# ben-hayes/neural-waveshaping-synthesis

Measured on AMD Instinct MI355X. Metric: audio_samples_per_sec, higher is better.
Workload: dtype f32 (fp16x2-split MFMA contractions = 22-bit products, fp32 accumulate; FiLM interpolation bf16x3-split MFMA = exact fp32 operands); 1 GPU; NEWT forward, vn checkpoint, FastNEWT LUT, batch 64/GPU x 500 frames (4 s @ 16 kHz), torch.rand F0/control, RNG draws on device; batch_per_gpu=64, frames=500, samples_per_utterance=64000, parallelism=batch-shard x1, exciter_opts=0, streams=2

## Files before the change

include/nws_hip.h:

```cpp
#ifndef NWS_HIP_H
#define NWS_HIP_H

#include <stddef.h>
#include <stdint.h>

#ifdef __cplusplus
extern "C" {
#endif

#define NWS_ABI_VERSION 6

#define NWS_N_HARMONICS 101
#define NWS_N_SHAPERS 64
#define NWS_HIDDEN 128
#define NWS_HOP 128
#define NWS_FIR_LEN 256
#define NWS_N_BANDS 129
#define NWS_FIR_HALF 128
#define NWS_SHAPER_WIDTH 8
#define NWS_FILM_CH 256

enum {
  NWS_OK = 0,
  NWS_ERR_UNSUPPORTED = -1,
// ... 85 lines not shown
#define NWS_MLP_FRAGS_BYTES 1474560
int nws_mlp_frags(const NwsWeights* w, const float* fir_design , void* frags_out, void* stream);

int nws_fir_design_matrix(const float* window , float* D_out, void* stream);

#define NWS_SPEC_ROW 132
#define NWS_MLP_SPEC_BYTES 200704
#define NWS_MLP_SPEC_FOLD_FLOATS 49668
int nws_fir_spectrum_map(const float* fir_design , double* S_out );
int nws_mlp_spec_fold(const float* proj_w, const float* proj_b, const float* newt_w0, const float* newt_b0, const float* hgen_w0,
                      const float* hgen_b0, const float* hgen_w3 , const float* hgen_b3 ,
                      const double* S , float* folded_out );
int nws_mlp_spec_frags(const float* folded , void* frags , void* stream);
int nws_frame_mlps_spec_serves(const NwsWeights* w, int B, int T);
int nws_frame_mlps_spec(const NwsWeights* w, const float* gru_out, int B, int T, float* film_out, float* spec_out, void* stream);

int nws_fir_noise(const float* fir , const float* noise , const float* add_in ,
                  int B, int T, float* out , void* stream);
int nws_fir_noise_window(const float* fir, const float* noise, int noise_len, int origin, const float* add_in, int B, int T,
                         float* out, void* stream);
int nws_fir_noise_spec(const float* spec , const float* noise , const float* add_in ,
                       int B, int T, float* out , void* stream);

int nws_fir_noise_grad(const float* noise , const float* grad_out , int B, int T,
                       float* grad_fir , void* stream);
int nws_fir_from_h_grad(const float* grad_fir , const float* fir_design , int B, int T,
                        float* grad_H , void* stream);
int nws_sum_batch_time(const float* x , int B, int C, int T, float* out , void* stream);

typedef struct NwsReverbPlan {
// ... 369 lines not shown
```

include/nws_hip_debug.h:

```cpp
#ifndef NWS_HIP_DEBUG_H
#define NWS_HIP_DEBUG_H
#include "nws_hip.h"
#ifdef __cplusplus
extern "C" {
#endif

int nws_debug_frame_mlps_kernel(int mode);

int nws_debug_forward_spec(int on);

int nws_debug_queue_busy(int groups, int spin_us, float* sink , void* stream);

int nws_debug_generic_exciter_plan(const NwsGenericModel* model, int B, int T, int out[8]);

int nws_debug_generic_gru_plan(int hidden, int C_in, int out[4]);

#ifdef __cplusplus
}
#endif
#endif
```

neural-waveshaping-synthesis_amd/_lib.py:

```python
from __future__ import annotations

import ctypes as C
import os

_HERE = os.path.dirname(os.path.abspath(__file__))
LIB_PATH = os.path.join(_HERE, "libnws_hip.so")

PROBE_LIB_PATH = os.path.join(_HERE, "libnws_probe.so")

ABI_VERSION = 6
EXCITER_VALU_FILM = 1
EXCITER_ONE_TERM = 2
EXCITER_HYBRID = 4
EXCITER_HYBRID_W = 8
EXCITER_BANK_NOFRACT = 16
N_HARMONICS = 101
N_SHAPERS = 64
HIDDEN = 128
HOP = 128
FIR_LEN = 256
FIR_HALF = 128
MLP_FRAGS_BYTES = 1474560
MLP_SPEC_BYTES = 200704
MLP_SPEC_FOLD_FLOATS = 49668
# ... 117 lines not shown
    "nws_control_gru_state": (C.c_int, [C.POINTER(NwsWeights), _fp, C.c_int, C.c_int, C.c_int, _fp, _fp, _fp, _fp]),
    "nws_control_gru_carry": (C.c_int, [C.POINTER(NwsWeights), _fp, _fp, C.c_int, C.c_int, C.c_int, _fp, _fp, _fp]),
    "nws_control_gru_batched": (C.c_int, [C.POINTER(NwsWeights), _fp, C.c_int, C.c_int, C.c_int, _fp, _fp, _fp, _fp]),
    "nws_control_gru_grad_workspace_bytes": (C.c_size_t, [C.c_int, C.c_int, C.c_int]),
    "nws_control_gru_grad": (C.c_int, [C.POINTER(NwsWeights), _fp, C.c_int, C.c_int, C.c_int, _fp, _fp, _fp, _fp, _fp, _fp, _fp, _fp,
                                       _fp, _fp, _fp, C.c_size_t, _fp]),
    "nws_frame_mlps": (C.c_int, [C.POINTER(NwsWeights), _fp, _fp, C.c_int, C.c_int, _fp, _fp, _fp, _fp, _fp]),
    "nws_mlp_frags": (C.c_int, [C.POINTER(NwsWeights), _fp, _fp, _fp]),
    "nws_debug_frame_mlps_kernel": (C.c_int, [C.c_int]),
    "nws_debug_forward_spec": (C.c_int, [C.c_int]),
    "nws_fir_spectrum_map": (C.c_int, [_fp, _fp]),
    "nws_mlp_spec_fold": (C.c_int, [_fp, _fp, _fp, _fp, _fp, _fp, _fp, _fp, _fp, _fp]),
    "nws_mlp_spec_frags": (C.c_int, [_fp, _fp, _fp]),
    "nws_frame_mlps_spec_serves": (C.c_int, [C.POINTER(NwsWeights), C.c_int, C.c_int]),
    "nws_frame_mlps_spec": (C.c_int, [C.POINTER(NwsWeights), _fp, C.c_int, C.c_int, _fp, _fp, _fp]),
    "nws_fir_noise_spec": (C.c_int, [_fp, _fp, _fp, C.c_int, C.c_int, _fp, _fp]),
    "nws_fir_design_matrix": (C.c_int, [_fp, _fp, _fp]),
    "nws_fir_noise": (C.c_int, [_fp, _fp, _fp, C.c_int, C.c_int, _fp, _fp]),
    "nws_fir_noise_window": (C.c_int, [_fp, _fp, C.c_int, C.c_int, _fp, C.c_int, C.c_int, _fp, _fp]),
    "nws_fir_noise_grad": (C.c_int, [_fp, _fp, C.c_int, C.c_int, _fp, _fp]),
    "nws_fir_from_h_grad": (C.c_int, [_fp, _fp, C.c_int, C.c_int, _fp, _fp]),
    "nws_sum_batch_time": (C.c_int, [_fp, C.c_int, C.c_int, C.c_int, _fp, _fp]),
    "nws_reverb_linear_chunk": (C.c_int, [C.POINTER(NwsReverbPlan), _fp, _fp, _fp, C.c_int, C.c_int, _fp, _fp, C.c_int, _fp, _fp,
                                          C.c_size_t, _fp]),
    "nws_reverb_plan": (C.c_int, [C.c_int, C.c_int, C.POINTER(NwsReverbPlan)]),
    "nws_reverb_plan_serves": (C.c_int, [C.POINTER(NwsReverbPlan), C.c_int, C.c_int]),
    "nws_reverb_table_bytes": (C.c_size_t, [C.POINTER(NwsReverbPlan)]),
    "nws_reverb_spectrum_bytes": (C.c_size_t, [C.POINTER(NwsReverbPlan)]),
    "nws_reverb_workspace_bytes": (C.c_size_t, [C.POINTER(NwsReverbPlan), C.c_int]),
    "nws_reverb_build_tables": (C.c_int, [C.POINTER(NwsReverbPlan), _fp, _fp]),
# ... 242 lines not shown
```

neural-waveshaping-synthesis_amd/build.py:

```python
import concurrent.futures as cf
import hashlib
import os
import subprocess
import sys

HERE = os.path.dirname(os.path.abspath(__file__))
CSRC = os.path.join(HERE, "csrc")
OBJ = os.path.join(HERE, "csrc", "_obj")
LIB = os.path.join(HERE, "libnws_hip.so")
OPS_LIB = os.path.join(HERE, "libnws_torch_ops.so")
PROBE_LIB = os.path.join(HERE, "libnws_probe.so")
SOURCES = ["exciter_newt.hip", "control_gru.hip", "control_gru_grad.hip", "frame_mlps.hip", "fir_noise.hip", "fir_noise_grad.hip", "reverb_fft.hip", "forward.hip",
           "loudness.hip", "loudness_stream.hip", "loudness_causal.hip", "mfcc.hip", "stft_loss.hip", "stft_grad.hip", "pyin.hip", "pyin_stream.hip", "resample.hip", "resample_stream.hip", "stages.hip", "td_mlp_grad.hip", "newt_grad.hip", "g_newt_grad.hip", "adam_step.hip", "generic.hip", "stream.hip", "queue_probe.hip", "exchange.hip", "grad_reduce.hip", "note_control.hip"]
PROBE_SOURCES = ["coexec_probe.hip"]
FLAGS = ["--offload-arch=gfx950", "-O3", "-std=c++17", "-ffp-contract=off", "-fPIC", "-fvisibility=default",
         "-Wall", "-Wno-unused-function", "-Wno-pass-failed", "-Rpass-analysis=kernel-resource-usage"]
KEEP_SLP = ("control_gru.hip",)
EXTRA_FLAGS = {src: ["-fno-slp-vectorize"] for src in SOURCES + PROBE_SOURCES if src not in KEEP_SLP}
FLAGS += [f for f in os.environ.get("NWS_EXTRA_HIPCC_FLAGS", "").split() if f]
LLVM_BIN = "/opt/rocm/lib/llvm/bin"
SWIZZLE_ALLOW = ("pk_probe_kernel", "pk_probe2_kernel", "pk_probe_mixed_kernel")


def _hipcc():
# ... 87 lines not shown
        else:
            window.append((1, set(), text))
        window = window[-8:]
    return found


REGISTER_BUDGETS = (
    ("exciter_newt_kernelILi4ELi2ELi2E", 80, "default oscillator kernel: three 8-wave workgroups per CU"),
    ("exciter_newt_kernelILi4ELi2ELi6E", 80, "one-term variant: three 8-wave workgroups per CU"),
    ("exciter_newt_kernelILi4ELi2ELi10E", 80, "hybrid variant: three 8-wave workgroups per CU"),
    ("exciter_newt_kernelILi4ELi2ELi26E", 80, "hybrid-W variant: three 8-wave workgroups per CU"),
    ("exciter_newt_kernelILi5ELi1ELi0E", 128, "exact-shaper bank kernel: four 4-wave workgroups per CU (38.8 KB of LDS each)"),
    ("exciter_newt_kernelILi6ELi1ELi0E", 128, "exact-shaper bank kernel (no v_fract): four 4-wave workgroups per CU"),
    ("g_exciter_newt_mfma_kernel", 128, "runtime-size oscillator kernel: four 4-wave workgroups per CU"),
)


def kernel_registers(remarks):
    regs, name = {}, None
    for line in remarks.splitlines():
        if "Function Name:" in line:
            name = line.split("Function Name:")[1].split("[-Rpass")[0].strip()
            regs[name] = 0
        elif name is not None and (" VGPRs:" in line or " AGPRs:" in line) and "Spill" not in line:
            regs[name] += int(line.split("GPRs:")[1].split()[0])
    return regs


def check_register_budgets(remarks, budgets=None):
    over = []
    for kernel, n in kernel_registers(remarks).items():
        for key, budget, why in (REGISTER_BUDGETS if budgets is None else budgets):
            if key in kernel and n > budget:
                over.append((kernel, n, budget, why))
    return over


def build_torch_ops(force=False, verbose=True):
    try:
        import torch
        from torch.utils import cpp_extension as ce
    except Exception as e:
        print(f"torch not importable ({e}): skipping libnws_torch_ops.so", file=sys.stderr)
        return None
    src = os.path.join(CSRC, "torch_ops.cpp")
    h = hashlib.sha256(open(src, "rb").read())
    h.update(open(os.path.join(HERE, "..", "include", "nws_hip.h"), "rb").read())
# ... 95 lines not shown
```

neural-waveshaping-synthesis_amd/csrc/forward.hip:

```cpp
#include "nws_common.h"

namespace {

struct Carve {
  char* p;
  size_t left;
  bool ok = true;
  void* take(size_t bytes) {
    bytes = (bytes + 255) & ~size_t(255);
    if (bytes > left) {
      ok = false;
      return nullptr;
    }
    void* r = p;
    p += bytes;
    left -= bytes;
    return r;
  }
};

size_t aligned(size_t b) { return (b + 255) & ~size_t(255); }

constexpr size_t kFirRow = NWS_SPEC_ROW > NWS_FIR_HALF ? NWS_SPEC_ROW : NWS_FIR_HALF;

// ... 71 lines not shown
                 const Arena& a, void* stream) {
  hipStream_t st = (hipStream_t)stream;
  int rc = NWS_OK;
  if (batched_gru) {
    NWS_STAGE(0, nws_phase_carry(f0, nullptr, B, T, a.carry, stream));
    NWS_STAGE(1, nws_control_gru_batched(w, control, B, C, T, nullptr, a.gru_out, nullptr, stream));
  } else {
    NWS_STAGE(0, NWS_OK);
    NWS_STAGE(1, nws_control_gru_carry(w, control, f0, B, C, T, a.gru_out, a.carry, stream));
  }
  return NWS_OK;
}

int audio_half(const NwsWeights* w, const NwsForwardAux* aux, const float* f0, int B, int T, float sample_rate,
               const float* phase_u, const float* rand_phase, const float* noise, float* out, const Arena& a, void* stream,
               void* wait_before_exciter = nullptr, void* record_after_exciter = nullptr, bool with_reverb = true) {
  hipStream_t st = (hipStream_t)stream;
  int rc = NWS_OK;
  const size_t N = (size_t)T * NWS_HOP;
  const bool spec = nws_frame_mlps_spec_serves(w, B, T) != 0;
  if (spec)
    NWS_STAGE(2, nws_frame_mlps_spec(w, a.gru_out, B, T, a.film, a.fir, stream));
  else
    NWS_STAGE(2, nws_frame_mlps(w, a.gru_out, aux->fir_design, B, T, nullptr, a.film, nullptr, a.fir, stream));
  if (spec)
    NWS_STAGE(4, nws_fir_noise_spec(a.fir, noise, nullptr, B, T, a.noise_out, stream));
  else
    NWS_STAGE(4, nws_fir_noise(a.fir, noise, nullptr, B, T, a.noise_out, stream));
  if (wait_before_exciter != nullptr) {
    const hipError_t e = hipStreamWaitEvent(st, (hipEvent_t)wait_before_exciter, 0);
    if (e != hipSuccess) return (int)e;
  }
  NWS_STAGE(3, nws_exciter_newt_add(w, f0, nullptr, a.carry, phase_u, rand_phase, a.film, a.noise_out, B, T, sample_rate, nullptr, a.pre, stream));
  if (record_after_exciter != nullptr) {
    const hipError_t e = hipEventRecord((hipEvent_t)record_after_exciter, st);
    if (e != hipSuccess) return (int)e;
  }
// ... 28 lines not shown
  const size_t N = (size_t)T * NWS_HOP;
  return aligned((size_t)B * (N / 32) * sizeof(double)) + aligned((size_t)B * T * NWS_HIDDEN * sizeof(float));
}

int nws_forward(const NwsWeights* w, const NwsForwardAux* aux, const float* f0, const float* control, int B, int C,
                int T, float sample_rate, const float* phase_u, const float* rand_phase, const float* noise, float* out,
                void* workspace, size_t workspace_bytes, void* stream) {
  if (!w || !aux_ok(aux)) return NWS_ERR_BAD_ARG;
  if (!f0 || !control || !phase_u || !rand_phase || !noise || !out || !workspace) return NWS_ERR_BAD_ARG;
  if (B <= 0 || T < 2 || C < 2) return NWS_ERR_BAD_ARG;
  if (T > (1 << 23) || !nws_reverb_plan_serves(aux->plan, T * NWS_HOP, 0)) return NWS_ERR_BAD_ARG;
  const Arena a = carve_arena(aux->plan, workspace, workspace_bytes, B, T, false);
  if (!a.ok) return NWS_ERR_WORKSPACE;
  const int rc = control_half(w, f0, control, B, C, T, 0, a, stream);
  if (rc != NWS_OK) return rc;
  return audio_half(w, aux, f0, B, T, sample_rate, phase_u, rand_phase, noise, out, a, stream);
}

int nws_forward_control(const NwsWeights* w, const float* f0, const float* control, int B, int C, int T, int batched_gru,
                        void* workspace, size_t workspace_bytes, void* stream) {
  if (!w || !f0 || !control || !workspace) return NWS_ERR_BAD_ARG;
  if (B <= 0 || T < 2 || C < 2) return NWS_ERR_BAD_ARG;
  const Arena a = carve_arena(nullptr, workspace, workspace_bytes, B, T, true);
  if (!a.ok) return NWS_ERR_WORKSPACE;
  return control_half(w, f0, control, B, C, T, batched_gru, a, stream);
}

int nws_forward_audio(const NwsWeights* w, const NwsForwardAux* aux, const float* f0, int B, int T, float sample_rate,
                      const float* phase_u, const float* rand_phase, const float* noise, float* out, void* workspace,
                      size_t workspace_bytes, void* stream) {
  if (!w || !aux_ok(aux)) return NWS_ERR_BAD_ARG;
// ... 116 lines not shown
```

neural-waveshaping-synthesis_amd/csrc/frame_mlps.hip:

```cpp
#include <cstdlib>

#include "nws_common.h"
#include "mlp_few.h"

namespace {

constexpr int kFT = 32;
constexpr int kXS = 33;
constexpr int kPS = 36;
constexpr int kRows = 132;
constexpr int kDK = 132;
constexpr float kLnEps = 1e-5f;

struct MlpLds {
  float emb[kRows * kXS];
  float p0[kRows * kXS];
  float p1[kRows * kXS];
  float stage[4][kFT * kPS];
  float red[2][4][kFT];
};

template <int KH>
__device__ __forceinline__ void gemm_tile(const float* __restrict__ W, int ldw, int row0, int n_rows,
                                          const float* __restrict__ X, int lane, f32x16& acc) {
// ... 691 lines not shown
  wr_split2(y[2], y[3], h1, l1);
  wr_split2(y[4], y[5], h2, l2);
  wr_split2(y[6], y[7], h3, l3);
  hi = f16x8{h0.x, h0.y, h1.x, h1.y, h2.x, h2.y, h3.x, h3.y};
  lo = f16x8{l0.x, l0.y, l1.x, l1.y, l2.x, l2.y, l3.x, l3.y};
}

__device__ __forceinline__ const char* wr_spec_chunk(const char* frags, int path, int k) {
  if (k == 0) return frags + kT3Base + (size_t)path * 65536;
  if (k == 1) return frags + kT2Base + (size_t)(path ? kT2Kb[1][2] : kT2Kb[0][2]) * 1024;
  if (k == 2) return frags + kT2Base + (size_t)(path ? kT2Kb[1][3] : kT2Kb[0][3]) * 1024;
  if (k == 3) return path ? frags + kT3Base + 131072 : frags + kT2Base + (size_t)kT2Kb[0][4] * 1024;
  return frags + kT2Base + (size_t)kT2Kb[0][5] * 1024;
}

__device__ __forceinline__ void wr_dma(const char* __restrict__ src, char* dst, int kb, int wave, int lane) {
  typedef __attribute__((address_space(1))) const void* gptr_t;
  typedef __attribute__((address_space(3))) void* lptr_t;
  const int per = kb * 128;
  const char* s = src + wave * per + lane * 16;
  char* d = dst + wave * per;
#pragma unroll
  for (int j = 0; j < 8; ++j) __builtin_amdgcn_global_load_lds((gptr_t)(s + j * 1024), (lptr_t)(d + j * 1024), 16, 0, 0);
  if (kb == 72) __builtin_amdgcn_global_load_lds((gptr_t)(s + 8192), (lptr_t)(d + 8192), 16, 0, 0);
}

template <int KS, int NMT, bool TRANSPOSED, bool ZERO = false>
__device__ __forceinline__ void wr_layer_mma(const char* slot, int mt0, const WrAct& x, f32x16* acc, int lane) {
  const char* a = slot + (size_t)mt0 * KS * 2048 + lane * 16;
  constexpr int S = KS * NMT;
  f16x8 wh[3], wl[3];
  auto ld = [&](int s2, int b) {
    const int mt = s2 % NMT, ks = s2 / NMT;
    wh[b] = *reinterpret_cast<const f16x8*>(a + (mt * KS + ks) * 2048);
    wl[b] = *reinterpret_cast<const f16x8*>(a + (mt * KS + ks) * 2048 + 1024);
  };
  ld(0, 0);
  if (S > 1) ld(1, 1);
  __builtin_amdgcn_sched_barrier(0x6);
  __builtin_amdgcn_s_setprio(2);
#pragma unroll
  for (int s2 = 0; s2 < S; ++s2) {
    const int mt = s2 % NMT, ks = s2 / NMT, b = s2 % 3;
    if (s2 + 2 < S) ld(s2 + 2, (s2 + 2) % 3);
    __builtin_amdgcn_sched_barrier(0x6);
    if (!TRANSPOSED) {
      acc[mt] = __builtin_amdgcn_mfma_f32_32x32x16_f16(wh[b], x.lo[ks], (ZERO && ks == 0) ? f32x16{} : acc[mt], 0, 0, 0);
      acc[mt] = __builtin_amdgcn_mfma_f32_32x32x16_f16(wl[b], x.hi[ks], acc[mt], 0, 0, 0);
      acc[mt] = __builtin_amdgcn_mfma_f32_32x32x16_f16(wh[b], x.hi[ks], acc[mt], 0, 0, 0);
    } else {
      acc[mt] = __builtin_amdgcn_mfma_f32_32x32x16_f16(x.lo[ks], wh[b], (ZERO && ks == 0) ? f32x16{} : acc[mt], 0, 0, 0);
      acc[mt] = __builtin_amdgcn_mfma_f32_32x32x16_f16(x.hi[ks], wl[b], acc[mt], 0, 0, 0);
      acc[mt] = __builtin_amdgcn_mfma_f32_32x32x16_f16(x.hi[ks], wh[b], acc[mt], 0, 0, 0);
    }
    __builtin_amdgcn_sched_barrier(0x6);
  }
  __builtin_amdgcn_s_setprio(0);
}

// ... 10 lines not shown
    }
}

__device__ __forceinline__ void wr_pack(const f32x16 (&v)[4], WrAct& out) {
#pragma unroll
  for (int mt = 0; mt < 4; ++mt)
#pragma unroll
    for (int g = 0; g < 2; ++g) {
      float y[8];
#pragma unroll
      for (int i = 0; i < 8; ++i) y[i] = v[mt][8 * g + i];
      wr_pack8(y, out.hi[2 * mt + g], out.lo[2 * mt + g]);
    }
}

__device__ __forceinline__ void wr_layer_norm(f32x16 (&v)[4], const float* g, const float* bt, int half) {
  float s0 = 0.0f, s1 = 0.0f, s2 = 0.0f, s3 = 0.0f;
#pragma unroll
  for (int r = 0; r < 16; ++r) {
    s0 += v[0][r];
    s1 += v[1][r];
    s2 += v[2][r];
    s3 += v[3][r];
  }
  float s = (s0 + s1) + (s2 + s3);
  s += nws_swap_halves(s);
  const float mean = s * (1.0f / NWS_HIDDEN);
  float q0 = 0.0f, q1 = 0.0f, q2 = 0.0f, q3 = 0.0f;
#pragma unroll
  for (int r = 0; r < 16; ++r) {
    v[0][r] -= mean;
    v[1][r] -= mean;
    v[2][r] -= mean;
    v[3][r] -= mean;
    q0 = fmaf(v[0][r], v[0][r], q0);
    q1 = fmaf(v[1][r], v[1][r], q1);
    q2 = fmaf(v[2][r], v[2][r], q2);
    q3 = fmaf(v[3][r], v[3][r], q3);
  }
  float q = (q0 + q1) + (q2 + q3);
  q += nws_swap_halves(q);
  const float rstd = 1.0f / sqrtf(q * (1.0f / NWS_HIDDEN) + kLnEps);
#pragma unroll
  for (int mt = 0; mt < 4; ++mt)
#pragma unroll
    for (int qd = 0; qd < 4; ++qd) {
      const int c = 32 * mt + 8 * qd + 4 * half;
      const float4 g4 = *reinterpret_cast<const float4*>(g + c), b4 = *reinterpret_cast<const float4*>(bt + c);
      const float gg[4] = {g4.x, g4.y, g4.z, g4.w}, bb[4] = {b4.x, b4.y, b4.z, b4.w};
#pragma unroll
      for (int i = 0; i < 4; ++i) {
        const float y = fmaf(v[mt][4 * qd + i] * rstd, gg[i], bb[i]);
        v[mt][4 * qd + i] = fmaxf(y, 0.01f * y);
      }
    }
}

template <int LD, bool BIAS>
__device__ __forceinline__ void wr_store_rows(__amdgpu_buffer_rsrc_t out, const f32x16& acc, int lane_off, int tile, float bias) {
#pragma unroll
  for (int r = 0; r < 16; ++r)
    __builtin_amdgcn_raw_buffer_store_b32(__builtin_bit_cast(unsigned, BIAS ? acc[r] + bias : acc[r]), out,
                                          lane_off + ((r & 3) * LD + 32 * tile) * 4, 8 * (r >> 2) * LD * 4, 0);
}

template <bool TAPS, bool SPEC = false>
__global__ __launch_bounds__(512, 2) void frame_mlps_wr_kernel(NwsWeights w, const float* __restrict__ gru_out, int F, int T,
                                                                 float* __restrict__ emb_out, float* __restrict__ film_out,
                                                                 float* __restrict__ H_out, float* __restrict__ fir_out,
                                                                 const int xcd_blocks = 0) {
  static_assert(!(TAPS && SPEC), "the folded form has neither an embedding nor H to store");
  extern __shared__ __attribute__((aligned(16))) char smem_raw[];
  WrLds& L = *reinterpret_cast<WrLds*>(smem_raw);
  const int tid = threadIdx.x, lane = tid & 63;
  const int wave = __builtin_amdgcn_readfirstlane(tid >> 6);
  const int fb = xcd_blocks > 0 ? (int)(blockIdx.x >> 4) * 8 + (int)(blockIdx.x & 7) : (int)blockIdx.x;
  const int path = xcd_blocks > 0 ? (int)((blockIdx.x >> 3) & 1) : (int)blockIdx.y;
  if (xcd_blocks > 0 && fb >= xcd_blocks) return;
  const int half = lane >> 5, col = lane & 31;
  const int f0 = fb * kWrFrames + 32 * wave;
  const int frame = f0 + col;
  const char* const frags = static_cast<const char*>(w.mlp_frags);
  const char* T2 = frags + kT2Base;
  const float* const spar = reinterpret_cast<const float*>(frags + kT3Base + kT3ParKb * 1024);
  char* const S0 = L.slot[0];
  char* const S1 = L.slot[1];

  wr_dma(SPEC ? wr_spec_chunk(frags, path, 0) : T2 + (size_t)kT2Kb[0][0] * 1024, S0, 64, wave, lane);
  const int grp = wave >> 1, pc = tid & 127;
  float pv[4];
  {
    auto sel4 = [&](const float* a, const float* b, const float* c, const float* d) { return grp == 0 ? a : grp == 1 ? b : grp == 2 ? c : d; };
    const float* const hb0 = SPEC ? spar + 128 * path : path ? w.hgen_b[0] : w.newt_mlp_b[0];
    const float* const hg0 = path ? w.hgen_ln_g[0] : w.newt_ln_g[0];
    const float* const ht0 = path ? w.hgen_ln_b[0] : w.newt_ln_b[0];
    const float* const hb1 = path ? w.hgen_b[1] : w.newt_mlp_b[1];
    const float* const hg1 = path ? w.hgen_ln_g[1] : w.newt_ln_g[1];
    const float* const ht1 = path ? w.hgen_ln_b[1] : w.newt_ln_b[1];
    const float* const hb2 = path ? w.hgen_b[2] : w.newt_mlp_b[2];
    const float* const hg2 = path ? w.hgen_ln_g[2] : w.newt_ln_g[2];
    const float* const ht2 = path ? w.hgen_ln_b[2] : w.newt_ln_b[2];
    const float* const ob = path ? (SPEC ? spar + 256 : w.hgen_b[3]) : w.newt_mlp_b[3];
    const float* const ox = path ? (SPEC ? spar + 384 : w.hgen_w[3] + (size_t)128 * NWS_HIDDEN) : w.newt_mlp_b[3] + 128;
    pv[0] = sel4(w.proj_b, hb0, hg0, ht0)[pc];
    pv[1] = sel4(hb1, hg1, ht1, hb2)[pc];
    pv[2] = sel4(hg2, ht2, ob, ox)[pc];
    pv[3] = w.proj_b[pc];
  }
  const float b128 = path ? (SPEC ? spar[512] : w.hgen_b[3][128]) : 0.0f;
  float4 in[16];
  {
    const float4* src = reinterpret_cast<const float4*>(gru_out + (size_t)(frame < F ? frame : F - 1) * NWS_HIDDEN + 64 * half);
#pragma unroll
    for (int k = 0; k < 16; ++k) in[k] = src[k];
  }
  L.par[128 * grp + pc] = pv[0];
  L.par[128 * (4 + grp) + pc] = pv[1];
  L.par[128 * (8 + grp) + pc] = pv[2];
  if (grp == 0) L.par[pc] = pv[3];
  if (tid == 0) L.par[1536] = b128;
  WrAct X;
#pragma unroll
  for (int ks = 0; ks < 8; ++ks) {
    const float y[8] = {in[2 * ks].x, in[2 * ks].y, in[2 * ks].z, in[2 * ks].w, in[2 * ks + 1].x, in[2 * ks + 1].y, in[2 * ks + 1].z, in[2 * ks + 1].w};
    wr_pack8(y, X.hi[ks], X.lo[ks]);
  }
  __builtin_amdgcn_sched_barrier(0);
  wr_dma(SPEC ? wr_spec_chunk(frags, path, 1) : T2 + (size_t)(path ? kT2Kb[1][1] : kT2Kb[0][1]) * 1024, S1, 64, wave, lane);
  __builtin_amdgcn_sched_barrier(0);
  auto sync = [&](int k) {
    if (k == 0) asm volatile("s_waitcnt vmcnt(8)" ::: "memory");
    else asm volatile("s_waitcnt vmcnt(0)" ::: "memory");
    asm volatile("s_waitcnt lgkmcnt(0)\n\ts_barrier" ::: "memory");
    if (SPEC) {
      if (k >= 1 && k + 1 <= (path ? 3 : 4)) wr_dma(wr_spec_chunk(frags, path, k + 1), ((k + 1) & 1) ? S1 : S0, 64, wave, lane);
    } else if (k >= 1 && k <= 4) {
      wr_dma(T2 + (size_t)(path ? kT2Kb[1][k + 1] : kT2Kb[0][k + 1]) * 1024, ((k + 1) & 1) ? S1 : S0, (path == 1 && k == 4) ? 72 : 64, wave, lane);
    }
  };
  sync(0);

  f32x16 v[4];
  if constexpr (!SPEC) {
    wr_lane_vec(L.par, half, v);
    wr_layer_mma<8, 4, false, false>(S0, 0, X, v, lane);
    if (TAPS && path == 0 && emb_out != nullptr && frame < F) {
      const int b = frame / T, t = frame - b * T;
#pragma unroll
      for (int mt = 0; mt < 4; ++mt)
#pragma unroll
        for (int r = 0; r < 16; ++r) emb_out[((size_t)b * NWS_HIDDEN + 32 * mt + nws_frag_row(r, half)) * T + t] = v[mt][r];
    }
    wr_pack(v, X);
    sync(1);
  }

  float h128 = 0.0f;
#pragma unroll
  for (int l = 0; l < 3; ++l) {
    const float* par = L.par + 128 + 384 * l;
    const char* slot = ((l & 1) != 0) != SPEC ? S0 : S1;
    wr_lane_vec(par, half, v);
    wr_layer_mma<8, 4, false, false>(slot, 0, X, v, lane);
    wr_layer_norm(v, par + 128, par + 256, half);
    if (l == 2 && path == 1) {
      f32x16 w128[4];
      wr_lane_vec(L.par + 1408, half, w128);
      float d0 = 0.0f, d1 = 0.0f, d2 = 0.0f, d3 = 0.0f;
#pragma unroll
      for (int r = 0; r < 16; ++r) {
        d0 = fmaf(v[0][r], w128[0][r], d0);
        d1 = fmaf(v[1][r], w128[1][r], d1);
        d2 = fmaf(v[2][r], w128[2][r], d2);
        d3 = fmaf(v[3][r], w128[3][r], d3);
      }
      float d = (d0 + d1) + (d2 + d3);
      d += nws_swap_halves(d);
      h128 = d + L.par[1536];
    }
    wr_pack(v, X);
    sync(SPEC ? l + 1 : l + 2);
  }

  if (path == 0) {
    const __amdgpu_buffer_rsrc_t film_rs = __builtin_amdgcn_make_buffer_rsrc(film_out, 0, F * NWS_FILM_CH * 4, 0x00020000);
    const int lane_off = ((f0 + 4 * half) * NWS_FILM_CH + col) * 4;
#pragma unroll
    for (int c = 0; c < 2; ++c) {
      const char* slot = (c != 0) != SPEC ? S1 : S0;
#pragma unroll
      for (int pr = 0; pr < 2; ++pr) {
        f32x16 acc[2];
        wr_layer_mma<8, 2, true, true>(slot, 2 * pr, X, acc, lane);
#pragma unroll
        for (int j = 0; j < 2; ++j)
          wr_store_rows<NWS_FILM_CH, true>(film_rs, acc[j], lane_off, 4 * c + 2 * pr + j, L.par[1280 + 32 * (4 * c + 2 * pr + j) + col]);
      }
      if (c == 0) sync(SPEC ? 4 : 5);
    }
  } else if constexpr (SPEC) {
    const __amdgpu_buffer_rsrc_t g_rs = __builtin_amdgcn_make_buffer_rsrc(fir_out, 0, F * NWS_SPEC_ROW * 4, 0x00020000);
    const int lane_off = ((f0 + 4 * half) * NWS_SPEC_ROW + col) * 4;
#pragma unroll
    for (int pr = 0; pr < 2; ++pr) {
      f32x16 acc[2];
      wr_layer_mma<8, 2, true, true>(S1, 2 * pr, X, acc, lane);
#pragma unroll
      for (int j = 0; j < 2; ++j) wr_store_rows<NWS_SPEC_ROW, true>(g_rs, acc[j], lane_off, 2 * pr + j, L.par[1280 + 32 * (2 * pr + j) + col]);
    }
    if (half == 0 && frame < F) fir_out[(size_t)frame * NWS_SPEC_ROW + 128] = h128;
  } else {
    wr_lane_vec(L.par + 1280, half, v);
    wr_layer_mma<8, 4, false, false>(S0, 0, X, v, lane);
    if (TAPS && H_out != nullptr && frame < F) {
#pragma unroll
      for (int mt = 0; mt < 4; ++mt)
#pragma unroll
        for (int r = 0; r < 16; ++r) H_out[(size_t)frame * NWS_N_BANDS + 32 * mt + nws_frag_row(r, half)] = v[mt][r];
      if (half == 0) H_out[(size_t)frame * NWS_N_BANDS + 128] = h128;
    }
    wr_pack(v, X);
    {
      const float y[8] = {half == 0 ? h128 : 0.0f, 0.0f, 0.0f, 0.0f, 0.0f, 0.0f, 0.0f, 0.0f};
      wr_pack8(y, X.hi[8], X.lo[8]);
    }
    sync(5);
    const __amdgpu_buffer_rsrc_t fir_rs = __builtin_amdgcn_make_buffer_rsrc(fir_out, 0, F * NWS_FIR_HALF * 4, 0x00020000);
    const int lane_off = ((f0 + 4 * half) * NWS_FIR_HALF + col) * 4;
#pragma unroll
    for (int pr = 0; pr < 2; ++pr) {
      f32x16 acc[2];
      wr_layer_mma<9, 2, true, true>(S1, 2 * pr, X, acc, lane);
#pragma unroll
      for (int j = 0; j < 2; ++j) wr_store_rows<NWS_FIR_HALF, false>(fir_rs, acc[j], lane_off, 2 * pr + j, 0.0f);
    }
  }
}

__global__ void mlp_frags2_kernel(NwsWeights w, const float* __restrict__ fir_design, f16x8* __restrict__ out) {
  constexpr int kPairs[10] = {2048, 2048, 2048, 2048, 4096, 2048, 2048, 2048, 2048, 2304};
  constexpr int kKb[10] = {0, 64, 128, 192, 256, 384, 448, 512, 576, 640};
  int e = blockIdx.x * blockDim.x + threadIdx.x;
  int id = 0;
  while (id < 10 && e >= kPairs[id]) e -= kPairs[id++];
  if (id >= 10) return;
  const int KS = id == 9 ? 9 : 8;
  const int li = e & 63, ks = (e >> 6) % KS, mt = (e >> 6) / KS;
// ... 200 lines not shown
}

static bool wr_kernel_serves(const NwsWeights* w, int B, int T) {
  const long long F = (long long)B * T;
  const bool many = (long long)B * ((T + kFT2 - 1) / kFT2) > 256;
  return w->mlp_frags != nullptr && g_mlp_kernel_mode != 1 && (many || g_mlp_kernel_mode == 2) &&
         F * NWS_FILM_CH * (long long)sizeof(float) < (1ll << 31);
}

static bool spec_serves(const NwsWeights* w, int B, int T) {
  return w && B >= 16 && B <= 65535 && T > 0 && w->mlp_spec != 0 && wr_kernel_serves(w, B, T);
}

int nws_frame_mlps_spec_serves(const NwsWeights* w, int B, int T) { return g_forward_spec && spec_serves(w, B, T) ? 1 : 0; }

int nws_frame_mlps_spec(const NwsWeights* w, const float* gru_out, int B, int T, float* film_out, float* spec_out, void* stream) {
  if (!w || !gru_out || !film_out || !spec_out || B <= 0 || T <= 0) return NWS_ERR_BAD_ARG;
  for (int i = 0; i < 4; ++i)
    if (!w->newt_mlp_w[i] || !w->newt_mlp_b[i] || !w->hgen_w[i] || !w->hgen_b[i]) return NWS_ERR_BAD_ARG;
  for (int i = 0; i < 3; ++i)
    if (!w->newt_ln_g[i] || !w->newt_ln_b[i] || !w->hgen_ln_g[i] || !w->hgen_ln_b[i]) return NWS_ERR_BAD_ARG;
  if (!w->proj_b) return NWS_ERR_BAD_ARG;
  if (!spec_serves(w, B, T)) return NWS_ERR_UNSUPPORTED;
  static unsigned long long attr_devices = 0;
  if (nws_first_use_on_device(attr_devices)) {
    const hipError_t e = hipFuncSetAttribute(reinterpret_cast<const void*>(frame_mlps_wr_kernel<false, true>),
                                             hipFuncAttributeMaxDynamicSharedMemorySize, (int)sizeof(WrLds));
    if (e != hipSuccess) return (int)e;
  }
  const long long F = (long long)B * T;
  const unsigned nblk = (unsigned)((F + kWrFrames - 1) / kWrFrames);
  const dim3 gridw(16 * ((nblk + 7) / 8), 1);
  frame_mlps_wr_kernel<false, true><<<gridw, 512, sizeof(WrLds), (hipStream_t)stream>>>(*w, gru_out, (int)F, T, nullptr, film_out, nullptr,
                                                                                         spec_out, (int)nblk);
  NWS_CHECK_LAUNCH();
  return NWS_OK;
}

static bool few_frames_enabled() {
  static const bool on = [] {
    const char* e = getenv("NWS_MLP_FEW");
    return e == nullptr || e[0] != '0';
  }();
  return on;
}

int nws_frame_mlps(const NwsWeights* w, const float* gru_out, const float* fir_design, int B, int T, float* emb_out,
                   float* film_out, float* H_out, float* fir_out, void* stream) {
  if (!w || !gru_out || !fir_design || !film_out || !fir_out || B <= 0 || T <= 0) return NWS_ERR_BAD_ARG;
  if (!w->proj_w || !w->proj_b) return NWS_ERR_BAD_ARG;
  for (int i = 0; i < 4; ++i)
// ... 100 lines not shown
```

Before: 10.72 billion samples/s.

## Add 12-wave folded frame-MLP kernel variant when sharing CUs with recurrence

Templates the folded frame-MLP kernel on waves per workgroup and adds a 12-wave, 384-frame-per-block variant. It uses a single-stage weight prefetch, a resplit DMA pattern, and a serialized layer norm to stay under a 168-register budget. A host heuristic picks 12 waves when the kernel runs beside the GRU recurrence and the CUs left free cannot hold all 8-wave blocks in one pass but can hold the 12-wave blocks. The aim is to avoid a second tail wave of blocks on the remaining CUs. The cost is shallower prefetch and fewer waves per SIMD.

```diff
diff --git a/include/nws_hip.h b/include/nws_hip.h
--- a/include/nws_hip.h
+++ b/include/nws_hip.h
@@ -123,6 +123,9 @@
 int nws_mlp_spec_frags(const float* folded , void* frags , void* stream);
 int nws_frame_mlps_spec_serves(const NwsWeights* w, int B, int T);
 int nws_frame_mlps_spec(const NwsWeights* w, const float* gru_out, int B, int T, float* film_out, float* spec_out, void* stream);
+int nws_frame_mlps_spec_beside(const NwsWeights* w, const float* gru_out, int B, int T, float* film_out, float* spec_out,
+                               int beside_recurrence, void* stream);
+int nws_frame_mlps_spec_waves(const NwsWeights* w, int B, int T, int beside_recurrence);
 
 int nws_fir_noise(const float* fir , const float* noise , const float* add_in ,
                   int B, int T, float* out , void* stream);
diff --git a/include/nws_hip_debug.h b/include/nws_hip_debug.h
--- a/include/nws_hip_debug.h
+++ b/include/nws_hip_debug.h
@@ -9,6 +9,12 @@
 
 int nws_debug_forward_spec(int on);
 
+int nws_debug_frame_mlps_waves(int waves);
+int nws_debug_frame_mlps_last_waves(void);
+
+int nws_debug_frame_mlps_spec_waves(const NwsWeights* w, const float* gru_out, int F, float* film_out, float* spec_out, int waves,
+                                    void* stream);
+
 int nws_debug_queue_busy(int groups, int spin_us, float* sink , void* stream);
 
 int nws_debug_generic_exciter_plan(const NwsGenericModel* model, int B, int T, int out[8]);
diff --git a/neural-waveshaping-synthesis_amd/_lib.py b/neural-waveshaping-synthesis_amd/_lib.py
--- a/neural-waveshaping-synthesis_amd/_lib.py
+++ b/neural-waveshaping-synthesis_amd/_lib.py
@@ -155,6 +155,11 @@
     "nws_mlp_spec_frags": (C.c_int, [_fp, _fp, _fp]),
     "nws_frame_mlps_spec_serves": (C.c_int, [C.POINTER(NwsWeights), C.c_int, C.c_int]),
     "nws_frame_mlps_spec": (C.c_int, [C.POINTER(NwsWeights), _fp, C.c_int, C.c_int, _fp, _fp, _fp]),
+    "nws_frame_mlps_spec_beside": (C.c_int, [C.POINTER(NwsWeights), _fp, C.c_int, C.c_int, _fp, _fp, C.c_int, _fp]),
+    "nws_frame_mlps_spec_waves": (C.c_int, [C.POINTER(NwsWeights), C.c_int, C.c_int, C.c_int]),
+    "nws_debug_frame_mlps_waves": (C.c_int, [C.c_int]),
+    "nws_debug_frame_mlps_last_waves": (C.c_int, []),
+    "nws_debug_frame_mlps_spec_waves": (C.c_int, [C.POINTER(NwsWeights), _fp, C.c_int, _fp, _fp, C.c_int, _fp]),
     "nws_fir_noise_spec": (C.c_int, [_fp, _fp, _fp, C.c_int, C.c_int, _fp, _fp]),
     "nws_fir_design_matrix": (C.c_int, [_fp, _fp, _fp]),
     "nws_fir_noise": (C.c_int, [_fp, _fp, _fp, C.c_int, C.c_int, _fp, _fp]),
diff --git a/neural-waveshaping-synthesis_amd/build.py b/neural-waveshaping-synthesis_amd/build.py
--- a/neural-waveshaping-synthesis_amd/build.py
+++ b/neural-waveshaping-synthesis_amd/build.py
@@ -125,6 +125,9 @@
     ("exciter_newt_kernelILi6ELi1ELi0E", 128, "exact-shaper bank kernel (no v_fract): four 4-wave workgroups per CU"),
     ("g_exciter_newt_mfma_kernel", 128, "runtime-size oscillator kernel: four 4-wave workgroups per CU"),
 )
+REGISTER_BUDGETS_FRAME_MLPS = (
+    ("frame_mlps_wr_kernelILb0ELb1ELi12E", 168, "12-wave folded frame-MLP kernel: three waves per SIMD"),
+)
 
 
 def kernel_registers(remarks):
@@ -141,7 +144,7 @@
 def check_register_budgets(remarks, budgets=None):
     over = []
     for kernel, n in kernel_registers(remarks).items():
-        for key, budget, why in (REGISTER_BUDGETS if budgets is None else budgets):
+        for key, budget, why in (REGISTER_BUDGETS + REGISTER_BUDGETS_FRAME_MLPS if budgets is None else budgets):
             if key in kernel and n > budget:
                 over.append((kernel, n, budget, why))
     return over
diff --git a/neural-waveshaping-synthesis_amd/csrc/forward.hip b/neural-waveshaping-synthesis_amd/csrc/forward.hip
--- a/neural-waveshaping-synthesis_amd/csrc/forward.hip
+++ b/neural-waveshaping-synthesis_amd/csrc/forward.hip
@@ -109,13 +109,14 @@
 
 int audio_half(const NwsWeights* w, const NwsForwardAux* aux, const float* f0, int B, int T, float sample_rate,
                const float* phase_u, const float* rand_phase, const float* noise, float* out, const Arena& a, void* stream,
-               void* wait_before_exciter = nullptr, void* record_after_exciter = nullptr, bool with_reverb = true) {
+               void* wait_before_exciter = nullptr, void* record_after_exciter = nullptr, bool with_reverb = true,
+               bool apart_from_control = true) {
   hipStream_t st = (hipStream_t)stream;
   int rc = NWS_OK;
   const size_t N = (size_t)T * NWS_HOP;
   const bool spec = nws_frame_mlps_spec_serves(w, B, T) != 0;
   if (spec)
-    NWS_STAGE(2, nws_frame_mlps_spec(w, a.gru_out, B, T, a.film, a.fir, stream));
+    NWS_STAGE(2, nws_frame_mlps_spec_beside(w, a.gru_out, B, T, a.film, a.fir, apart_from_control ? 1 : 0, stream));
   else
     NWS_STAGE(2, nws_frame_mlps(w, a.gru_out, aux->fir_design, B, T, nullptr, a.film, nullptr, a.fir, stream));
   if (spec)
@@ -174,7 +175,7 @@
   if (!a.ok) return NWS_ERR_WORKSPACE;
   const int rc = control_half(w, f0, control, B, C, T, 0, a, stream);
   if (rc != NWS_OK) return rc;
-  return audio_half(w, aux, f0, B, T, sample_rate, phase_u, rand_phase, noise, out, a, stream);
+  return audio_half(w, aux, f0, B, T, sample_rate, phase_u, rand_phase, noise, out, a, stream, nullptr, nullptr, true, false);
 }
 
 int nws_forward_control(const NwsWeights* w, const float* f0, const float* control, int B, int C, int T, int batched_gru,
diff --git a/neural-waveshaping-synthesis_amd/csrc/frame_mlps.hip b/neural-waveshaping-synthesis_amd/csrc/frame_mlps.hip
--- a/neural-waveshaping-synthesis_amd/csrc/frame_mlps.hip
+++ b/neural-waveshaping-synthesis_amd/csrc/frame_mlps.hip
@@ -729,9 +729,21 @@
   return frags + kT2Base + (size_t)kT2Kb[0][5] * 1024;
 }
 
+constexpr int kWrDmaMin12 = 5;
+template <int NW>
 __device__ __forceinline__ void wr_dma(const char* __restrict__ src, char* dst, int kb, int wave, int lane) {
   typedef __attribute__((address_space(1))) const void* gptr_t;
   typedef __attribute__((address_space(3))) void* lptr_t;
+  static_assert(NW == 8 || NW == 12, "waves per workgroup");
+  if constexpr (NW == 12) {
+    const char* s = src + wave * 1024 + lane * 16;
+    char* d = dst + wave * 1024;
+#pragma unroll
+    for (int j = 0; j < kWrDmaMin12; ++j) __builtin_amdgcn_global_load_lds((gptr_t)(s + j * 12288), (lptr_t)(d + j * 12288), 16, 0, 0);
+    if (kWrDmaMin12 * 12 + wave < kb)
+      __builtin_amdgcn_global_load_lds((gptr_t)(s + kWrDmaMin12 * 12288), (lptr_t)(d + kWrDmaMin12 * 12288), 16, 0, 0);
+    return;
+  }
   const int per = kb * 128;
   const char* s = src + wave * per + lane * 16;
   char* d = dst + wave * per;
@@ -740,24 +752,24 @@
   if (kb == 72) __builtin_amdgcn_global_load_lds((gptr_t)(s + 8192), (lptr_t)(d + 8192), 16, 0, 0);
 }
 
-template <int KS, int NMT, bool TRANSPOSED, bool ZERO = false>
+template <int KS, int NMT, bool TRANSPOSED, bool ZERO = false, int PF = 2>
 __device__ __forceinline__ void wr_layer_mma(const char* slot, int mt0, const WrAct& x, f32x16* acc, int lane) {
   const char* a = slot + (size_t)mt0 * KS * 2048 + lane * 16;
   constexpr int S = KS * NMT;
-  f16x8 wh[3], wl[3];
+  f16x8 wh[PF + 1], wl[PF + 1];
   auto ld = [&](int s2, int b) {
     const int mt = s2 % NMT, ks = s2 / NMT;
     wh[b] = *reinterpret_cast<const f16x8*>(a + (mt * KS + ks) * 2048);
     wl[b] = *reinterpret_cast<const f16x8*>(a + (mt * KS + ks) * 2048 + 1024);
   };
   ld(0, 0);
-  if (S > 1) ld(1, 1);
+  if (S > 1 && PF > 1) ld(1, 1);
   __builtin_amdgcn_sched_barrier(0x6);
   __builtin_amdgcn_s_setprio(2);
 #pragma unroll
   for (int s2 = 0; s2 < S; ++s2) {
-    const int mt = s2 % NMT, ks = s2 / NMT, b = s2 % 3;
-    if (s2 + 2 < S) ld(s2 + 2, (s2 + 2) % 3);
+    const int mt = s2 % NMT, ks = s2 / NMT, b = s2 % (PF + 1);
+    if (s2 + PF < S) ld(s2 + PF, (s2 + PF) % (PF + 1));
     __builtin_amdgcn_sched_barrier(0x6);
     if (!TRANSPOSED) {
       acc[mt] = __builtin_amdgcn_mfma_f32_32x32x16_f16(wh[b], x.lo[ks], (ZERO && ks == 0) ? f32x16{} : acc[mt], 0, 0, 0);
@@ -798,6 +810,7 @@
     }
 }
 
+template <bool SEQ = false>
 __device__ __forceinline__ void wr_layer_norm(f32x16 (&v)[4], const float* g, const float* bt, int half) {
   float s0 = 0.0f, s1 = 0.0f, s2 = 0.0f, s3 = 0.0f;
 #pragma unroll
@@ -825,8 +838,16 @@
   float q = (q0 + q1) + (q2 + q3);
   q += nws_swap_halves(q);
   const float rstd = 1.0f / sqrtf(q * (1.0f / NWS_HIDDEN) + kLnEps);
-#pragma unroll
-  for (int mt = 0; mt < 4; ++mt)
+  if (SEQ) {
+    int ho = 4 * half;
+    asm volatile("" : "+v"(ho));
+    g += ho;
+    bt += ho;
+    half = 0;
+  }
+#pragma unroll
+  for (int mt = 0; mt < 4; ++mt) {
+    if (SEQ) __builtin_amdgcn_sched_barrier(0);
 #pragma unroll
     for (int qd = 0; qd < 4; ++qd) {
       const int c = 32 * mt + 8 * qd + 4 * half;
@@ -838,6 +859,9 @@
         v[mt][4 * qd + i] = fmaxf(y, 0.01f * y);
       }
     }
+    if (SEQ) asm volatile("" : "+v"(v[mt]));
+  }
+  if (SEQ) __builtin_amdgcn_sched_barrier(0);
 }
 
 template <int LD, bool BIAS>
@@ -848,12 +872,14 @@
                                           lane_off + ((r & 3) * LD + 32 * tile) * 4, 8 * (r >> 2) * LD * 4, 0);
 }
 
-template <bool TAPS, bool SPEC = false>
-__global__ __launch_bounds__(512, 2) void frame_mlps_wr_kernel(NwsWeights w, const float* __restrict__ gru_out, int F, int T,
-                                                                 float* __restrict__ emb_out, float* __restrict__ film_out,
-                                                                 float* __restrict__ H_out, float* __restrict__ fir_out,
-                                                                 const int xcd_blocks = 0) {
+template <bool TAPS, bool SPEC = false, int NW = 8>
+__global__ __launch_bounds__(64 * NW, NW / 4) void frame_mlps_wr_kernel(NwsWeights w, const float* __restrict__ gru_out, int F, int T,
+                                                                          float* __restrict__ emb_out, float* __restrict__ film_out,
+                                                                          float* __restrict__ H_out, float* __restrict__ fir_out,
+                                                                          const int xcd_blocks = 0) {
   static_assert(!(TAPS && SPEC), "the folded form has neither an embedding nor H to store");
+  static_assert(NW == 8 || (NW == 12 && SPEC), "12 waves: the folded form only");
+  constexpr int PF = NW == 8 ? 2 : 1;
   extern __shared__ __attribute__((aligned(16))) char smem_raw[];
   WrLds& L = *reinterpret_cast<WrLds*>(smem_raw);
   const int tid = threadIdx.x, lane = tid & 63;
@@ -862,7 +888,7 @@
   const int path = xcd_blocks > 0 ? (int)((blockIdx.x >> 3) & 1) : (int)blockIdx.y;
   if (xcd_blocks > 0 && fb >= xcd_blocks) return;
   const int half = lane >> 5, col = lane & 31;
-  const int f0 = fb * kWrFrames + 32 * wave;
+  const int f0 = fb * (32 * NW) + 32 * wave;
   const int frame = f0 + col;
   const char* const frags = static_cast<const char*>(w.mlp_frags);
   const char* T2 = frags + kT2Base;
@@ -870,10 +896,11 @@
   char* const S0 = L.slot[0];
   char* const S1 = L.slot[1];
 
-  wr_dma(SPEC ? wr_spec_chunk(frags, path, 0) : T2 + (size_t)kT2Kb[0][0] * 1024, S0, 64, wave, lane);
+  wr_dma<NW>(SPEC ? wr_spec_chunk(frags, path, 0) : T2 + (size_t)kT2Kb[0][0] * 1024, S0, 64, wave, lane);
   const int grp = wave >> 1, pc = tid & 127;
-  float pv[4];
-  {
+  const bool fetches = NW == 8 || grp < 4;
+  float pv[4] = {0.0f, 0.0f, 0.0f, 0.0f};
+  if (fetches) {
     auto sel4 = [&](const float* a, const float* b, const float* c, const float* d) { return grp == 0 ? a : grp == 1 ? b : grp == 2 ? c : d; };
     const float* const hb0 = SPEC ? spar + 128 * path : path ? w.hgen_b[0] : w.newt_mlp_b[0];
     const float* const hg0 = path ? w.hgen_ln_g[0] : w.newt_ln_g[0];
@@ -898,9 +925,11 @@
 #pragma unroll
     for (int k = 0; k < 16; ++k) in[k] = src[k];
   }
-  L.par[128 * grp + pc] = pv[0];
-  L.par[128 * (4 + grp) + pc] = pv[1];
-  L.par[128 * (8 + grp) + pc] = pv[2];
+  if (fetches) {
+    L.par[128 * grp + pc] = pv[0];
+    L.par[128 * (4 + grp) + pc] = pv[1];
+    L.par[128 * (8 + grp) + pc] = pv[2];
+  }
   if (grp == 0) L.par[pc] = pv[3];
   if (tid == 0) L.par[1536] = b128;
   WrAct X;
@@ -910,16 +939,18 @@
     wr_pack8(y, X.hi[ks], X.lo[ks]);
   }
   __builtin_amdgcn_sched_barrier(0);
-  wr_dma(SPEC ? wr_spec_chunk(frags, path, 1) : T2 + (size_t)(path ? kT2Kb[1][1] : kT2Kb[0][1]) * 1024, S1, 64, wave, lane);
+  wr_dma<NW>(SPEC ? wr_spec_chunk(frags, path, 1) : T2 + (size_t)(path ? kT2Kb[1][1] : kT2Kb[0][1]) * 1024, S1, 64, wave, lane);
   __builtin_amdgcn_sched_barrier(0);
   auto sync = [&](int k) {
-    if (k == 0) asm volatile("s_waitcnt vmcnt(8)" ::: "memory");
+    if (k == 0 && NW == 8) asm volatile("s_waitcnt vmcnt(8)" ::: "memory");
+    else if (k == 0 && wave < 64 - 12 * kWrDmaMin12) asm volatile("s_waitcnt vmcnt(6)" ::: "memory");
+    else if (k == 0) asm volatile("s_waitcnt vmcnt(5)" ::: "memory");
     else asm volatile("s_waitcnt vmcnt(0)" ::: "memory");
     asm volatile("s_waitcnt lgkmcnt(0)\n\ts_barrier" ::: "memory");
     if (SPEC) {
-      if (k >= 1 && k + 1 <= (path ? 3 : 4)) wr_dma(wr_spec_chunk(frags, path, k + 1), ((k + 1) & 1) ? S1 : S0, 64, wave, lane);
+      if (k >= 1 && k + 1 <= (path ? 3 : 4)) wr_dma<NW>(wr_spec_chunk(frags, path, k + 1), ((k + 1) & 1) ? S1 : S0, 64, wave, lane);
     } else if (k >= 1 && k <= 4) {
-      wr_dma(T2 + (size_t)(path ? kT2Kb[1][k + 1] : kT2Kb[0][k + 1]) * 1024, ((k + 1) & 1) ? S1 : S0, (path == 1 && k == 4) ? 72 : 64, wave, lane);
+      wr_dma<NW>(T2 + (size_t)(path ? kT2Kb[1][k + 1] : kT2Kb[0][k + 1]) * 1024, ((k + 1) & 1) ? S1 : S0, (path == 1 && k == 4) ? 72 : 64, wave, lane);
     }
   };
   sync(0);
@@ -927,7 +958,7 @@
   f32x16 v[4];
   if constexpr (!SPEC) {
     wr_lane_vec(L.par, half, v);
-    wr_layer_mma<8, 4, false, false>(S0, 0, X, v, lane);
+    wr_layer_mma<8, 4, false, false, PF>(S0, 0, X, v, lane);
     if (TAPS && path == 0 && emb_out != nullptr && frame < F) {
       const int b = frame / T, t = frame - b * T;
 #pragma unroll
@@ -945,8 +976,8 @@
     const float* par = L.par + 128 + 384 * l;
     const char* slot = ((l & 1) != 0) != SPEC ? S0 : S1;
     wr_lane_vec(par, half, v);
-    wr_layer_mma<8, 4, false, false>(slot, 0, X, v, lane);
-    wr_layer_norm(v, par + 128, par + 256, half);
+    wr_layer_mma<8, 4, false, false, PF>(slot, 0, X, v, lane);
+    wr_layer_norm<NW == 12>(v, par + 128, par + 256, half);
     if (l == 2 && path == 1) {
       f32x16 w128[4];
       wr_lane_vec(L.par + 1408, half, w128);
@@ -963,6 +994,11 @@
       h128 = d + L.par[1536];
     }
     wr_pack(v, X);
+    if constexpr (NW == 12) {
+#pragma unroll
+      for (int ks = 0; ks < 8; ++ks) asm volatile("" : "+v"(X.hi[ks]), "+v"(X.lo[ks]));
+      __builtin_amdgcn_sched_barrier(0);
+    }
     sync(SPEC ? l + 1 : l + 2);
   }
 
@@ -975,7 +1011,7 @@
 #pragma unroll
       for (int pr = 0; pr < 2; ++pr) {
         f32x16 acc[2];
-        wr_layer_mma<8, 2, true, true>(slot, 2 * pr, X, acc, lane);
+        wr_layer_mma<8, 2, true, true, PF>(slot, 2 * pr, X, acc, lane);
 #pragma unroll
         for (int j = 0; j < 2; ++j)
           wr_store_rows<NWS_FILM_CH, true>(film_rs, acc[j], lane_off, 4 * c + 2 * pr + j, L.par[1280 + 32 * (4 * c + 2 * pr + j) + col]);
@@ -988,14 +1024,14 @@
 #pragma unroll
     for (int pr = 0; pr < 2; ++pr) {
       f32x16 acc[2];
-      wr_layer_mma<8, 2, true, true>(S1, 2 * pr, X, acc, lane);
+      wr_layer_mma<8, 2, true, true, PF>(S1, 2 * pr, X, acc, lane);
 #pragma unroll
       for (int j = 0; j < 2; ++j) wr_store_rows<NWS_SPEC_ROW, true>(g_rs, acc[j], lane_off, 2 * pr + j, L.par[1280 + 32 * (2 * pr + j) + col]);
     }
     if (half == 0 && frame < F) fir_out[(size_t)frame * NWS_SPEC_ROW + 128] = h128;
   } else {
     wr_lane_vec(L.par + 1280, half, v);
-    wr_layer_mma<8, 4, false, false>(S0, 0, X, v, lane);
+    wr_layer_mma<8, 4, false, false, PF>(S0, 0, X, v, lane);
     if (TAPS && H_out != nullptr && frame < F) {
 #pragma unroll
       for (int mt = 0; mt < 4; ++mt)
@@ -1014,7 +1050,7 @@
 #pragma unroll
     for (int pr = 0; pr < 2; ++pr) {
       f32x16 acc[2];
-      wr_layer_mma<9, 2, true, true>(S1, 2 * pr, X, acc, lane);
+      wr_layer_mma<9, 2, true, true, PF>(S1, 2 * pr, X, acc, lane);
 #pragma unroll
       for (int j = 0; j < 2; ++j) wr_store_rows<NWS_FIR_HALF, false>(fir_rs, acc[j], lane_off, 2 * pr + j, 0.0f);
     }
@@ -1245,27 +1281,94 @@
 
 int nws_frame_mlps_spec_serves(const NwsWeights* w, int B, int T) { return g_forward_spec && spec_serves(w, B, T) ? 1 : 0; }
 
-int nws_frame_mlps_spec(const NwsWeights* w, const float* gru_out, int B, int T, float* film_out, float* spec_out, void* stream) {
-  if (!w || !gru_out || !film_out || !spec_out || B <= 0 || T <= 0) return NWS_ERR_BAD_ARG;
-  for (int i = 0; i < 4; ++i)
-    if (!w->newt_mlp_w[i] || !w->newt_mlp_b[i] || !w->hgen_w[i] || !w->hgen_b[i]) return NWS_ERR_BAD_ARG;
-  for (int i = 0; i < 3; ++i)
-    if (!w->newt_ln_g[i] || !w->newt_ln_b[i] || !w->hgen_ln_g[i] || !w->hgen_ln_b[i]) return NWS_ERR_BAD_ARG;
-  if (!w->proj_b) return NWS_ERR_BAD_ARG;
-  if (!spec_serves(w, B, T)) return NWS_ERR_UNSUPPORTED;
+static int device_cus() {
+  static int cus[64] = {};
+  int d = 0;
+  if (hipGetDevice(&d) != hipSuccess || d < 0 || d > 63) return 0;
+  if (cus[d] == 0) {
+    int n = 0;
+    if (hipDeviceGetAttribute(&n, hipDeviceAttributeMultiprocessorCount, d) != hipSuccess || n <= 0) return 0;
+    cus[d] = n;
+  }
+  return cus[d];
+}
+
+static int g_spec_waves = 0;
+static int g_spec_last_waves = 0;
+static int spec_waves(int B, int T, bool beside_recurrence) {
+  if (g_spec_waves != 0) return g_spec_waves;
+  if (!beside_recurrence) return 8;
+  const long long F = (long long)B * T;
+  const long long left = (long long)device_cus() - B;
+  return (2 * ((F + 255) / 256) > left && left >= 2 * ((F + 383) / 384)) ? 12 : 8;
+}
+
+int nws_debug_frame_mlps_waves(int waves) {
+  if (waves != 0 && waves != 8 && waves != 12) return NWS_ERR_BAD_ARG;
+  g_spec_waves = waves;
+  return NWS_OK;
+}
+
+int nws_debug_frame_mlps_last_waves(void) { return g_spec_last_waves; }
+
+int nws_frame_mlps_spec_waves(const NwsWeights* w, int B, int T, int beside_recurrence) {
+  return nws_frame_mlps_spec_serves(w, B, T) ? spec_waves(B, T, beside_recurrence != 0) : 0;
+}
+
+static int launch_wr_spec(const NwsWeights* w, const float* gru_out, long long F, int T, float* film_out, float* spec_out, int waves,
+                          void* stream) {
+  if (waves == 12 && F > (1ll << 20)) return NWS_ERR_UNSUPPORTED;
   static unsigned long long attr_devices = 0;
   if (nws_first_use_on_device(attr_devices)) {
-    const hipError_t e = hipFuncSetAttribute(reinterpret_cast<const void*>(frame_mlps_wr_kernel<false, true>),
-                                             hipFuncAttributeMaxDynamicSharedMemorySize, (int)sizeof(WrLds));
+    hipError_t e = hipFuncSetAttribute(reinterpret_cast<const void*>(frame_mlps_wr_kernel<false, true>),
+                                       hipFuncAttributeMaxDynamicSharedMemorySize, (int)sizeof(WrLds));
     if (e != hipSuccess) return (int)e;
-  }
-  const long long F = (long long)B * T;
-  const unsigned nblk = (unsigned)((F + kWrFrames - 1) / kWrFrames);
+    e = hipFuncSetAttribute(reinterpret_cast<const void*>(frame_mlps_wr_kernel<false, true, 12>),
+                            hipFuncAttributeMaxDynamicSharedMemorySize, (int)sizeof(WrLds));
+    if (e != hipSuccess) return (int)e;
+  }
+  const int per = 32 * waves;
+  const unsigned nblk = (unsigned)((F + per - 1) / per);
   const dim3 gridw(16 * ((nblk + 7) / 8), 1);
-  frame_mlps_wr_kernel<false, true><<<gridw, 512, sizeof(WrLds), (hipStream_t)stream>>>(*w, gru_out, (int)F, T, nullptr, film_out, nullptr,
-                                                                                         spec_out, (int)nblk);
+  if (waves == 12)
+    frame_mlps_wr_kernel<false, true, 12><<<gridw, 768, sizeof(WrLds), (hipStream_t)stream>>>(*w, gru_out, (int)F, T, nullptr, film_out,
+                                                                                               nullptr, spec_out, (int)nblk);
+  else
+    frame_mlps_wr_kernel<false, true><<<gridw, 512, sizeof(WrLds), (hipStream_t)stream>>>(*w, gru_out, (int)F, T, nullptr, film_out, nullptr,
+                                                                                           spec_out, (int)nblk);
   NWS_CHECK_LAUNCH();
+  g_spec_last_waves = waves;
   return NWS_OK;
+}
+
+static bool spec_weights_ok(const NwsWeights* w) {
+  if (!w || !w->proj_b) return false;
+  for (int i = 0; i < 4; ++i)
+    if (!w->newt_mlp_w[i] || !w->newt_mlp_b[i] || !w->hgen_w[i] || !w->hgen_b[i]) return false;
+  for (int i = 0; i < 3; ++i)
+    if (!w->newt_ln_g[i] || !w->newt_ln_b[i] || !w->hgen_ln_g[i] || !w->hgen_ln_b[i]) return false;
+  return true;
+}
+
+int nws_frame_mlps_spec_beside(const NwsWeights* w, const float* gru_out, int B, int T, float* film_out, float* spec_out,
+                               int beside_recurrence, void* stream) {
+  if (!w || !gru_out || !film_out || !spec_out || B <= 0 || T <= 0) return NWS_ERR_BAD_ARG;
+  if (!spec_weights_ok(w)) return NWS_ERR_BAD_ARG;
+  if (!spec_serves(w, B, T)) return NWS_ERR_UNSUPPORTED;
+  return launch_wr_spec(w, gru_out, (long long)B * T, T, film_out, spec_out, spec_waves(B, T, beside_recurrence != 0), stream);
+}
+
+int nws_frame_mlps_spec(const NwsWeights* w, const float* gru_out, int B, int T, float* film_out, float* spec_out, void* stream) {
+  return nws_frame_mlps_spec_beside(w, gru_out, B, T, film_out, spec_out, 0, stream);
+}
+
+int nws_debug_frame_mlps_spec_waves(const NwsWeights* w, const float* gru_out, int F, float* film_out, float* spec_out, int waves,
+                                    void* stream) {
+  if (!w || !gru_out || !film_out || !spec_out || F <= 0 || (waves != 8 && waves != 12)) return NWS_ERR_BAD_ARG;
+  if (!spec_weights_ok(w)) return NWS_ERR_BAD_ARG;
+  if (w->mlp_frags == nullptr || w->mlp_spec == 0 || (long long)F * NWS_FILM_CH * (long long)sizeof(float) >= (1ll << 31))
+    return NWS_ERR_UNSUPPORTED;
+  return launch_wr_spec(w, gru_out, F, F, film_out, spec_out, waves, stream);
 }
 
 static bool few_frames_enabled() {
```

New measurement: 10.85 billion samples/s (median of 6 runs). 1.01x the previous value.
